# r9y9/gantts

Measured on NVIDIA H100. Metric: gan_step_frames_per_sec, higher is better.
Workload: dtype f32 (GEMMs: bf16x3 split on wgmma, fp32 accumulate)

## Files before the change

### gantts_b200/csrc/gemm_tc.cu

```cuda
#include <cuda.h>
#include <cuda_bf16.h>

#include "common.cuh"
#include "tc_ptx.cuh"

namespace gantts {

constexpr int TC_WG_WARPS = 4;
constexpr int TC_THREADS = 128 + 2 * 32 * TC_WG_WARPS;
constexpr int TC_BM = 128;
constexpr int TC_WARP_PITCH = 20;
constexpr int TC_WARP_BUF_FLOATS = 32 * TC_WARP_PITCH;
constexpr int TC_MAX_BN = 128;
constexpr int TC_KK_BK = 64;
constexpr int TC_MN_BK = 32;
constexpr int TC_MAX_STAGES = 8;
constexpr int TC_PRODUCER_REGS = 40;
constexpr int TC_CONSUMER_REGS = 232;
constexpr uint32_t TC_SMEM_MAX = 227 * 1024;
constexpr uint32_t TC_BIAS_SMEM = 4096;
constexpr uint32_t TC_ONES_SMEM = 1024;

constexpr int EPI_F32 = 0;
constexpr int EPI_PLANES_FWD = 1;
constexpr int EPI_PLANES_BWD = 2;

struct GemmParams {
  int64_t rows_a;
  int cols_b;
  int64_t red;
  int64_t red_chunk;
  int num_a, num_b, num_z;
  int bn;
  int num_stages;
  uint32_t stage_bytes, b_plane_bytes, tx_bytes;
  int64_t row0;
  uint32_t a_plane;
  uint32_t atom_bytes;
  uint32_t epi_off;
  uint32_t bar_off;
  float* C;
  int64_t ldc, c_zstride;
  int vec_ok;
  int accumulate;
  __nv_bfloat16 *out_hi, *out_lo;
  int64_t out_pitch;
  uint32_t* code;
  int64_t code_pitch;
  uint32_t bias_off;
  float* db;
  uint32_t ones_off;
  const float* bias;
  int act;
  float slope, keep_scale;
  uint32_t thresh;
  uint64_t seed;
};

__device__ __forceinline__ uint32_t pack_bf16x2(float a, float b) {
  __nv_bfloat162 h = __floats2bfloat162_rn(a, b);
  return *reinterpret_cast<uint32_t*>(&h);
}

__device__ __forceinline__ void split8(const float* v, uint32_t* h, uint32_t* l) {
#pragma unroll
  for (int i = 0; i < 4; ++i) {
    const float a = v[2 * i], b = v[2 * i + 1];
    const uint32_t hp = pack_bf16x2(a, b);
    const float ah = __uint_as_float(hp << 16), bh = __uint_as_float(hp & 0xffff0000u);
    h[i] = hp;
    l[i] = pack_bf16x2(a - ah, b - bh);
  }
}

__device__ __forceinline__ void store_planes16(const float* v, __nv_bfloat16* hi, __nv_bfloat16* lo, int col,
                                               int64_t pitch) {
  uint32_t h[8], l[8];
  split8(v, h, l);
  split8(v + 8, h + 4, l + 4);
  if (col + 16 <= pitch) {
    reinterpret_cast<uint4*>(hi)[0] = make_uint4(h[0], h[1], h[2], h[3]);
    reinterpret_cast<uint4*>(hi)[1] = make_uint4(h[4], h[5], h[6], h[7]);
    reinterpret_cast<uint4*>(lo)[0] = make_uint4(l[0], l[1], l[2], l[3]);
    reinterpret_cast<uint4*>(lo)[1] = make_uint4(l[4], l[5], l[6], l[7]);
  } else if (col + 8 <= pitch) {
    *reinterpret_cast<uint4*>(hi) = make_uint4(h[0], h[1], h[2], h[3]);
    *reinterpret_cast<uint4*>(lo) = make_uint4(l[0], l[1], l[2], l[3]);
  }
}

__device__ __forceinline__ void dropout16(float (&v)[16], uint64_t seed, uint32_t row, int n_cols, int col, uint32_t thresh,
                                          float scale) {
  const uint32_t quarter_n = (uint32_t)(n_cols + 3) >> 2, limit = drop_limit(thresh);
#pragma unroll
  for (int q = 0; q < 4; ++q) {
    const DropBits d = dropout_quad_bits(seed, row, quarter_n, ((uint32_t)col >> 2) + q);
    v[4 * q] = (d.a << 16) > limit ? v[4 * q] * scale : 0.f;
    v[4 * q + 1] = d.a > limit ? v[4 * q + 1] * scale : 0.f;
    v[4 * q + 2] = (d.b << 16) > limit ? v[4 * q + 2] * scale : 0.f;
    v[4 * q + 3] = d.b > limit ? v[4 * q + 3] * scale : 0.f;
  }
}

__device__ __forceinline__ void epilogue_f32_smem(const GemmParams& p, const uint32_t (&r)[16], int64_t row0,
                                                  int lane, int col, int z, const float* __restrict__ bias_s,
                                                  float* scr) {
  const int64_t row = row0 + (lane & 15);
  const int lcol = col + 16 * (lane >> 4);
  float v[16];
#pragma unroll
  for (int j = 0; j < 16; ++j) v[j] = __uint_as_float(r[j]);
  if (p.bias) {
    if (bias_s) {
#pragma unroll
      for (int j = 0; j < 16; ++j) v[j] += bias_s[lcol + j];
    } else {
#pragma unroll
      for (int j = 0; j < 16; ++j)
        if (lcol + j < p.cols_b) v[j] += __ldg(p.bias + lcol + j);
    }
  }
  if (p.act == GANTTS_ACT_LEAKY_DROPOUT) {
#pragma unroll
    for (int j = 0; j < 16; ++j) v[j] = fmaxf(v[j], v[j] * p.slope);
    if (p.thresh) dropout16(v, p.seed, (uint32_t)(row + p.row0), p.cols_b, lcol, p.thresh, p.keep_scale);
  } else if (p.act == GANTTS_ACT_SIGMOID) {
#pragma unroll
    for (int j = 0; j < 16; ++j) v[j] = 1.f / (1.f + expf(-v[j]));
  }
  const int sw = (lane >> 1) & 3;
#pragma unroll
  for (int k = 0; k < 4; ++k)
    *reinterpret_cast<float4*>(scr + lane * 16 + 4 * (k ^ sw)) = make_float4(v[4 * k], v[4 * k + 1], v[4 * k + 2], v[4 * k + 3]);
  __syncwarp();
  float* cbase = p.C + (int64_t)z * p.c_zstride;
  const int j = lane & 15, hr = lane >> 4;
#pragma unroll
  for (int h = 0; h < 2; ++h) {
    const int c = col + 16 * h + j;
    const bool col_ok = c < p.cols_b;
    float* q[8];
    bool ok[8];
    float old[8];
#pragma unroll
    for (int i = 0; i < 8; ++i) {
      const int64_t rw = row0 + 2 * i + hr;
      q[i] = cbase + c + rw * p.ldc;
      ok[i] = col_ok && rw < p.rows_a;
    }
    if (p.accumulate) {
#pragma unroll
      for (int i = 0; i < 8; ++i) old[i] = ok[i] ? __ldcg(q[i]) : 0.f;
    }
#pragma unroll
    for (int i = 0; i < 8; ++i) {
      const int rr = 2 * (8 * h + i) + hr;
      const float val = scr[rr * 16 + 4 * ((j >> 2) ^ ((rr >> 1) & 3)) + (j & 3)];
      if (ok[i]) *q[i] = p.accumulate ? old[i] + val : val;
    }
  }
  __syncwarp();
}

template <int EPI>
__device__ __forceinline__ uint32_t epilogue_chunk16(const GemmParams& p, const uint32_t (&r)[16], int64_t row,
                                                     int col, int z, const float* __restrict__ bias_s,
                                                     uint32_t code_in) {
  uint32_t code = 0;
  float v[16];
#pragma unroll
  for (int j = 0; j < 16; ++j) v[j] = __uint_as_float(r[j]);
  if (EPI == EPI_F32) {
    float* crow = p.C + (int64_t)z * p.c_zstride + row * p.ldc;
    if (p.bias) {
      if (bias_s) {
#pragma unroll
        for (int j = 0; j < 16; ++j) v[j] += bias_s[col + j];
      } else {
#pragma unroll
        for (int j = 0; j < 16; ++j)
          if (col + j < p.cols_b) v[j] += __ldg(p.bias + col + j);
      }
    }
    if (p.act == GANTTS_ACT_LEAKY_DROPOUT) {
#pragma unroll
      for (int j = 0; j < 16; ++j) v[j] = fmaxf(v[j], v[j] * p.slope);
      if (p.thresh) dropout16(v, p.seed, (uint32_t)(row + p.row0), p.cols_b, col, p.thresh, p.keep_scale);
    } else if (p.act == GANTTS_ACT_SIGMOID) {
#pragma unroll
      for (int j = 0; j < 16; ++j) v[j] = 1.f / (1.f + expf(-v[j]));
    }
#pragma unroll
    for (int j = 0; j < 16; j += 4) {
      const int c = col + j;
      if (c + 3 < p.cols_b) {
        *reinterpret_cast<float4*>(crow + c) = make_float4(v[j], v[j + 1], v[j + 2], v[j + 3]);
      } else {
#pragma unroll
        for (int e = 0; e < 4; ++e)
          if (c + e < p.cols_b) crow[c + e] = v[j + e];
      }
    }
  } else if (EPI == EPI_PLANES_FWD) {
    if (bias_s) {
#pragma unroll
      for (int j = 0; j < 16; j += 4) {
        const float4 b4 = *reinterpret_cast<const float4*>(bias_s + col + j);
        v[j] += b4.x; v[j + 1] += b4.y; v[j + 2] += b4.z; v[j + 3] += b4.w;
      }
    } else {
#pragma unroll
      for (int j = 0; j < 16; ++j)
        if (col + j < p.cols_b) v[j] += __ldg(p.bias + col + j);
    }
    if (p.thresh) {
      const uint32_t quarter_n = (uint32_t)(p.cols_b + 3) >> 2, limit = drop_limit(p.thresh);
      const uint32_t grow = (uint32_t)(row + p.row0);
#pragma unroll
      for (int q = 0; q < 4; ++q) {
        const DropBits d = dropout_quad_bits(p.seed, grow, quarter_n, ((uint32_t)col >> 2) + q);
#pragma unroll
        for (int e = 0; e < 4; ++e) {
          const int j = 4 * q + e;
          const uint32_t w = e < 2 ? d.a : d.b;
          const bool keep = ((e & 1) ? w : (w << 16)) > limit;
          const bool neg = v[j] < 0.f;
          const float a = neg ? v[j] * p.slope : v[j];
          v[j] = keep ? a * p.keep_scale : 0.f;
          if (!keep) code |= 1u << (2 * j);
          if (neg) code |= 2u << (2 * j);
        }
      }
    } else {
#pragma unroll
      for (int j = 0; j < 16; ++j) {
        const bool neg = v[j] < 0.f;
        v[j] = neg ? v[j] * p.slope : v[j];
        if (v[j] == 0.f) code |= 1u << (2 * j);
        if (neg) code |= 2u << (2 * j);
      }
    }
    __nv_bfloat16* oh = p.out_hi + row * p.out_pitch + col;
    __nv_bfloat16* ol = p.out_lo + row * p.out_pitch + col;
    store_planes16(v, oh, ol, col, p.out_pitch);
  } else {
    const float dpos = p.keep_scale, dneg = p.slope * p.keep_scale;
    const float dzero = p.thresh ? 0.f : p.slope;
#pragma unroll
    for (int j = 0; j < 16; ++j) {
      const uint32_t cj = (code_in >> (2 * j)) & 3u;
      v[j] *= (cj & 1u) ? dzero : ((cj & 2u) ? dneg : dpos);
    }
    __nv_bfloat16* oh = p.out_hi + row * p.out_pitch + col;
    __nv_bfloat16* ol = p.out_lo + row * p.out_pitch + col;
    store_planes16(v, oh, ol, col, p.out_pitch);
  }
  return code;
}

template <bool MN, int BN, bool DB>
__device__ __forceinline__ void mma_tile(const GemmParams& p, float (&acc)[BN / 2], float (&accdb)[4], uint32_t base,
                                         uint32_t full0, uint32_t empty0, uint64_t d_ones, int nk, uint32_t& s,
                                         uint32_t& ph, int lane, int blk) {
  constexpr int BK = MN ? TC_MN_BK : TC_KK_BK;
  constexpr uint32_t kstep = MN ? 2048u : 32u;
  const uint32_t a_half = MN ? p.atom_bytes : 8192u;
  const uint32_t a_off = (uint32_t)blk * a_half;
#pragma unroll
  for (int i = 0; i < BN / 2; ++i) acc[i] = 0.f;
  uint32_t prev = 0;
#pragma unroll 1
  for (int kb = 0; kb < nk; ++kb) {
    ptx::mbar_wait(full0 + 8 * s, ph);
    const uint32_t sa_hi = base + s * p.stage_bytes, sa_lo = sa_hi + p.a_plane;
    const uint32_t sb_hi = sa_lo + p.a_plane, sb_lo = sb_hi + p.b_plane_bytes;
    ptx::wgmma_fence();
#pragma unroll
    for (int k = 0; k < BK / 16; ++k) {
      const uint64_t db_hi = ptx::make_smem_desc(sb_hi + k * kstep, p.atom_bytes, 1024u);
      const uint64_t db_lo = ptx::make_smem_desc(sb_lo + k * kstep, p.atom_bytes, 1024u);
      const uint64_t da_hi = ptx::make_smem_desc(sa_hi + a_off + k * kstep, p.atom_bytes, 1024u);
      const uint64_t da_lo = ptx::make_smem_desc(sa_lo + a_off + k * kstep, p.atom_bytes, 1024u);
      if constexpr (BN == 128) {
        ptx::wgmma_m64n128k16<MN ? 1 : 0, MN ? 1 : 0>(acc, da_hi, db_hi);
        ptx::wgmma_m64n128k16<MN ? 1 : 0, MN ? 1 : 0>(acc, da_hi, db_lo);
        ptx::wgmma_m64n128k16<MN ? 1 : 0, MN ? 1 : 0>(acc, da_lo, db_hi);
      } else {
        ptx::wgmma_m64n64k16<MN ? 1 : 0, MN ? 1 : 0>(acc, da_hi, db_hi);
        ptx::wgmma_m64n64k16<MN ? 1 : 0, MN ? 1 : 0>(acc, da_hi, db_lo);
        ptx::wgmma_m64n64k16<MN ? 1 : 0, MN ? 1 : 0>(acc, da_lo, db_hi);
      }
      if constexpr (DB) {
        ptx::wgmma_m64n8k16<MN ? 1 : 0>(accdb, da_hi, d_ones);
        ptx::wgmma_m64n8k16<MN ? 1 : 0>(accdb, da_lo, d_ones);
      }
    }
    ptx::wgmma_commit();
    if (kb > 0) {
      ptx::wgmma_wait<1>();
      __syncwarp();
      if (lane == 0) ptx::mbar_arrive(empty0 + 8 * prev);
    }
    prev = s;
    if (++s == (uint32_t)p.num_stages) { s = 0; ph ^= 1; }
  }
  __syncwarp();
  ptx::wgmma_wait<0>();
  ptx::fence_regs(acc);
  ptx::fence_regs(accdb);
  __syncwarp();
  if (lane == 0) ptx::mbar_arrive(empty0 + 8 * prev);
}

template <bool MN, int EPI, int BN>
__global__ void __launch_bounds__(TC_THREADS, 1)
gemm_bf16x3_kernel(const __grid_constant__ CUtensorMap tmAh, const __grid_constant__ CUtensorMap tmAl,
                   const __grid_constant__ CUtensorMap tmBh, const __grid_constant__ CUtensorMap tmBl,
                   const GemmParams p) {
  constexpr int BK = MN ? TC_MN_BK : TC_KK_BK;
  extern __shared__ uint8_t smem_raw[];
  const uint32_t raw = ptx::smem_u32(smem_raw);
  const uint32_t base = (raw + 1023u) & ~1023u;
  uint8_t* const gbase = smem_raw + (base - raw);
  const uint32_t full0 = base + p.bar_off, empty0 = full0 + 8 * TC_MAX_STAGES;
  const int warp = threadIdx.x >> 5, lane = threadIdx.x & 31;
  const int tiles_ab = p.num_a * p.num_b;
  const int tiles = tiles_ab * p.num_z;
  auto k_blocks = [&](int z) {
    const int64_t r_beg = (int64_t)z * p.red_chunk;
    const int64_t r_end = r_beg + p.red_chunk < p.red ? r_beg + p.red_chunk : p.red;
    return (int)((r_end - r_beg + BK - 1) / BK);
  };

  if (threadIdx.x == 0) {
    for (int s = 0; s < p.num_stages; ++s) {
      ptx::mbar_init(full0 + 8 * s, 1);
      ptx::mbar_init(empty0 + 8 * s, 2 * TC_WG_WARPS);
    }
    ptx::fence_barrier_init();
    ptx::prefetch_tensormap(&tmAh);
    ptx::prefetch_tensormap(&tmAl);
    ptx::prefetch_tensormap(&tmBh);
    ptx::prefetch_tensormap(&tmBl);
  }
  ptx::pdl_launch_dependents();
  ptx::pdl_wait();
  const float* bias_s = nullptr;
  if (p.bias_off) {
    float* bs = reinterpret_cast<float*>(gbase + p.bias_off);
    const int nb = p.num_b * BN;
    for (int i = threadIdx.x; i < nb; i += TC_THREADS) bs[i] = i < p.cols_b ? p.bias[i] : 0.f;
    bias_s = bs;
  }
  if (MN && p.db != nullptr) {
    uint32_t* ones = reinterpret_cast<uint32_t*>(gbase + p.ones_off);
    for (int i = threadIdx.x; i < (int)(TC_ONES_SMEM / 4); i += TC_THREADS) ones[i] = 0x3F803F80u;
    ptx::fence_proxy_async();
  }
  __syncthreads();

  if (warp < 4) {
    ptx::setmaxnreg_dec<TC_PRODUCER_REGS>();
    if (threadIdx.x == 0) {
      uint32_t s = 0, ph = 0;
      for (int t = blockIdx.x; t < tiles; t += gridDim.x) {
        const int z = t / tiles_ab, rem = t - z * tiles_ab;
        const int a0 = (rem / p.num_b) * TC_BM, b0 = (rem % p.num_b) * BN;
        const int64_t r_beg = (int64_t)z * p.red_chunk;
        const int nk = k_blocks(z);
        for (int kb = 0; kb < nk; ++kb) {
          const int64_t r0 = r_beg + (int64_t)kb * BK;
          ptx::mbar_wait(empty0 + 8 * s, ph ^ 1);
          const uint32_t fb = full0 + 8 * s;
          ptx::mbar_expect_tx(fb, p.tx_bytes);
          const uint32_t sa_hi = base + s * p.stage_bytes, sa_lo = sa_hi + p.a_plane;
          const uint32_t sb_hi = sa_lo + p.a_plane, sb_lo = sb_hi + p.b_plane_bytes;
          if (!MN) {
            ptx::tma_load_2d(sa_hi, &tmAh, fb, (int32_t)r0, a0);
            ptx::tma_load_2d(sb_hi, &tmBh, fb, (int32_t)r0, b0);
            ptx::tma_load_2d(sa_lo, &tmAl, fb, (int32_t)r0, a0);
            ptx::tma_load_2d(sb_lo, &tmBl, fb, (int32_t)r0, b0);
          } else {
            for (int j = 0; j < TC_BM / 64; ++j) {
              ptx::tma_load_2d(sa_hi + j * p.atom_bytes, &tmAh, fb, a0 + 64 * j, (int32_t)r0);
              ptx::tma_load_2d(sa_lo + j * p.atom_bytes, &tmAl, fb, a0 + 64 * j, (int32_t)r0);
            }
            for (int j = 0; j < BN / 64; ++j) {
              ptx::tma_load_2d(sb_hi + j * p.atom_bytes, &tmBh, fb, b0 + 64 * j, (int32_t)r0);
              ptx::tma_load_2d(sb_lo + j * p.atom_bytes, &tmBl, fb, b0 + 64 * j, (int32_t)r0);
            }
          }
          if (++s == (uint32_t)p.num_stages) { s = 0; ph ^= 1; }
        }
      }
    }
    return;
  }

  ptx::setmaxnreg_inc<TC_CONSUMER_REGS>();
  const int wg = (warp >> 2) - 1;
  const int q = warp & 3;
  float* const wbuf = reinterpret_cast<float*>(gbase + p.epi_off) + (warp - 4) * TC_WARP_BUF_FLOATS;
  const uint64_t d_ones = ptx::make_smem_desc(base + p.ones_off, 0u, 1024u);
  uint32_t s = 0, ph = 0;
  for (int t = blockIdx.x; t < tiles; t += gridDim.x) {
    const int z = t / tiles_ab, rem = t - z * tiles_ab;
    const int nk = k_blocks(z);
    const int ta = rem / p.num_b, tb = rem % p.num_b;
    const int a0 = ta * TC_BM, b0 = tb * BN;
    float acc[BN / 2];
    float accdb[4] = {0.f, 0.f, 0.f, 0.f};
    const bool do_db = MN && p.db != nullptr && tb == 0;
    if (do_db)
      mma_tile<MN, BN, MN>(p, acc, accdb, base, full0, empty0, d_ones, nk, s, ph, lane, wg);
    else
      mma_tile<MN, BN, false>(p, acc, accdb, base, full0, empty0, d_ones, nk, s, ph, lane, wg);
    const int64_t row0 = (int64_t)a0 + 64 * wg + 16 * q;
    if (do_db && (lane & 3) == 0) {
      const int64_t r = row0 + (lane >> 2);
      if (r < p.rows_a) p.db[(int64_t)z * p.rows_a + r] = accdb[0];
      if (r + 8 < p.rows_a) p.db[(int64_t)z * p.rows_a + r + 8] = accdb[2];
    }
    const int64_t row = row0 + (lane & 15);
    const bool row_ok = row < p.rows_a;
    constexpr int PASSES = BN / 32;
    uint32_t codes[PASSES];
    uint32_t code_out[PASSES];
#pragma unroll
    for (int k = 0; k < PASSES; ++k) {
      const int c = b0 + 16 * (2 * k + (lane >> 4));
      codes[k] = code_out[k] = 0u;
      if (EPI == EPI_PLANES_BWD && row_ok && c < p.cols_b) codes[k] = __ldg(p.code + row * p.code_pitch + (c >> 4));
    }
#pragma unroll
    for (int k = 0; k < PASSES; ++k) {
      __syncwarp();
#pragma unroll
      for (int h = 0; h < 2; ++h)
#pragma unroll
        for (int jj = 0; jj < 2; ++jj) {
          const int j = 2 * (2 * k + h) + jj;
          float* w = wbuf + (16 * h + (lane >> 2)) * TC_WARP_PITCH + 8 * jj + 2 * (lane & 3);
          *reinterpret_cast<float2*>(w) = make_float2(acc[4 * j], acc[4 * j + 1]);
          *reinterpret_cast<float2*>(w + 8 * TC_WARP_PITCH) = make_float2(acc[4 * j + 2], acc[4 * j + 3]);
        }
      __syncwarp();
      uint32_t rr[16];
      const float4* src = reinterpret_cast<const float4*>(wbuf + lane * TC_WARP_PITCH);
#pragma unroll
      for (int m = 0; m < 4; ++m) {
        const float4 f = src[m];
        rr[4 * m] = __float_as_uint(f.x); rr[4 * m + 1] = __float_as_uint(f.y);
        rr[4 * m + 2] = __float_as_uint(f.z); rr[4 * m + 3] = __float_as_uint(f.w);
      }
      const int col = b0 + 32 * k;
      const int lcol = col + 16 * (lane >> 4);
      if (EPI == EPI_F32 && !p.vec_ok) {
        __syncwarp();
        if (col < p.cols_b) epilogue_f32_smem(p, rr, row0, lane, col, z, bias_s, wbuf);
      } else if (row_ok && lcol < p.cols_b) {
        code_out[k] = epilogue_chunk16<EPI>(p, rr, row, lcol, z, bias_s, codes[k]);
      }
    }
    if (EPI == EPI_PLANES_FWD && p.code != nullptr && row_ok) {
      uint32_t* cpp = p.code + row * p.code_pitch + (b0 >> 4);
#pragma unroll
      for (int k = 0; k < PASSES; ++k) {
        const int ck = 2 * k + (lane >> 4);
        if (b0 + 16 * ck < p.cols_b) cpp[ck] = code_out[k];
      }
    }
  }
}

__global__ void split_planes_kernel(const float* __restrict__ src, int64_t rs, int64_t rows, int cols,
                                    __nv_bfloat16* __restrict__ hi, __nv_bfloat16* __restrict__ lo,
                                    int64_t pitch, int transpose) {
  pdl_entry();
  const int lane = threadIdx.x & 31;
  const int64_t warp = ((int64_t)blockIdx.x * blockDim.x + threadIdx.x) >> 5;
  const int64_t nwarps = ((int64_t)gridDim.x * blockDim.x) >> 5;
  if (!transpose) {
    for (int64_t r = warp; r < rows; r += nwarps) {
      const float* sr = src + r * rs;
      uint32_t* hr = reinterpret_cast<uint32_t*>(hi + r * pitch);
      uint32_t* lr = reinterpret_cast<uint32_t*>(lo + r * pitch);
#pragma unroll 2
      for (int c = 2 * lane; c < cols; c += 64) {
        const float a = sr[c], b = (c + 1 < cols) ? sr[c + 1] : 0.f;
        const uint32_t hp = pack_bf16x2(a, b);
        const float ah = __uint_as_float(hp << 16), bh = __uint_as_float(hp & 0xffff0000u);
        hr[c >> 1] = hp;
        lr[c >> 1] = pack_bf16x2(a - ah, b - bh);
      }
    }
  } else {
    for (int64_t r = warp; r < rows; r += nwarps)
      for (int c = lane; c < cols; c += 32) {
        const float v = src[r * rs + c];
        const __nv_bfloat16 h = __float2bfloat16_rn(v);
        hi[(int64_t)c * pitch + r] = h;
        lo[(int64_t)c * pitch + r] = __float2bfloat16_rn(v - __bfloat162float(h));
      }
  }
}

__global__ void splitk_reduce_kernel(const float* __restrict__ partial, int nsplit, int64_t n,
                                     float* __restrict__ out, int accumulate);

typedef CUresult (*EncodeTiledFn)(CUtensorMap*, CUtensorMapDataType, cuuint32_t, void*, const cuuint64_t*,
                                  const cuuint64_t*, const cuuint32_t*, const cuuint32_t*,
                                  CUtensorMapInterleave, CUtensorMapSwizzle, CUtensorMapL2promotion,
                                  CUtensorMapFloatOOBfill);

static EncodeTiledFn get_encode() {
  static EncodeTiledFn fn = nullptr;
  if (!fn) {
    void* p = nullptr;
    cudaDriverEntryPointQueryResult q;
    if (cudaGetDriverEntryPoint("cuTensorMapEncodeTiled", &p, cudaEnableDefault, &q) == cudaSuccess &&
        q == cudaDriverEntryPointSuccess)
      fn = reinterpret_cast<EncodeTiledFn>(p);
  }
  return fn;
}

static int make_map(CUtensorMap* m, const void* ptr, int64_t rows, int64_t cols, int64_t pitch, int box_rows) {
  EncodeTiledFn enc = get_encode();
  if (!enc) {
    set_error("tc: cuTensorMapEncodeTiled entry point unavailable");
    return GANTTS_E_CUDA;
  }
  cuuint64_t dims[2] = {(cuuint64_t)cols, (cuuint64_t)rows};
  cuuint64_t strides[1] = {(cuuint64_t)pitch * 2};
  cuuint32_t box[2] = {64u, (cuuint32_t)box_rows};
  cuuint32_t estr[2] = {1, 1};
  CUresult r = enc(m, CU_TENSOR_MAP_DATA_TYPE_BFLOAT16, 2, const_cast<void*>(ptr), dims, strides, box, estr,
                   CU_TENSOR_MAP_INTERLEAVE_NONE, CU_TENSOR_MAP_SWIZZLE_128B,
                   CU_TENSOR_MAP_L2_PROMOTION_L2_256B,
                   CU_TENSOR_MAP_FLOAT_OOB_FILL_NONE);
  if (r != CUDA_SUCCESS) {
    set_error("tc: cuTensorMapEncodeTiled failed (%d) rows=%lld cols=%lld pitch=%lld box_rows=%d", (int)r,
              (long long)rows, (long long)cols, (long long)pitch, box_rows);
    return GANTTS_E_CUDA;
  }
  return GANTTS_OK;
}

static int current_device() {
  int dev = -1;
  if (cudaGetDevice(&dev) != cudaSuccess) return -1;
  return dev;
}

static int num_sms() {
  static int n[64] = {};
  const int dev = current_device();
  if (dev < 0 || dev >= 64) return 132;
  if (!n[dev]) {
    cudaDeviceGetAttribute(&n[dev], cudaDevAttrMultiProcessorCount, dev);
    if (n[dev] <= 0) n[dev] = 132;
  }
  return n[dev];
}

static inline int64_t pitch_for(int64_t cols) { return (cols + 15) / 16 * 16; }
static inline size_t plane_bytes(int64_t rows, int64_t cols) {
  return ((size_t)rows * pitch_for(cols) * 2 + 255) / 256 * 256;
}

struct Planes {
  __nv_bfloat16 *hi, *lo;
  int64_t rows, cols, pitch;
};

static Planes carve_planes(char*& cur, int64_t rows, int64_t cols) {
  Planes pl;
  pl.rows = rows;
  pl.cols = cols;
  pl.pitch = pitch_for(cols);
  pl.hi = reinterpret_cast<__nv_bfloat16*>(cur);
  cur += plane_bytes(rows, cols);
  pl.lo = reinterpret_cast<__nv_bfloat16*>(cur);
  cur += plane_bytes(rows, cols);
  return pl;
}

static int launch_split(const float* src, int64_t rs, int64_t rows, int cols, const Planes& pl, int transpose,
                        cudaStream_t st) {
  int64_t total = rows * cols;
  int nb = (int)((total + 1023) / 1024);
  if (nb > num_sms() * 8) nb = num_sms() * 8;
  if (nb < 1) nb = 1;
  GANTTS_PDL_LAUNCH((split_planes_kernel), nb, 256, 0, st, src, rs, rows, cols, pl.hi, pl.lo, pl.pitch, transpose);
  GANTTS_LAUNCH_CHECK("split_planes_kernel");
  return GANTTS_OK;
}

static int pick_bn(int n) {
  int bn = (n + 63) / 64 * 64;
  if (bn <= TC_MAX_BN) return bn;
  int tiles = (n + TC_MAX_BN - 1) / TC_MAX_BN;
  bn = ((n + tiles - 1) / tiles + 63) / 64 * 64;
  return bn;
}

struct EpiArgs {
  int epi = EPI_F32;
  float* C = nullptr;
  int64_t ldc = 0;
  int accumulate = 0;
  __nv_bfloat16 *out_hi = nullptr, *out_lo = nullptr;
  int64_t out_pitch = 0;
  uint32_t* code = nullptr;
  int64_t code_pitch = 0;
  const float* bias = nullptr;
  int act = GANTTS_ACT_NONE;
  float slope = 0.f, p = 0.f;
  uint64_t seed = 0;
  int64_t row0 = 0;
};

static void fill_epilogue(GemmParams& p, const EpiArgs& e) {
  p.C = e.C;
  p.ldc = e.ldc;
  p.accumulate = e.accumulate;
  p.vec_ok = (!e.accumulate && e.C && (e.ldc & 3) == 0 && (reinterpret_cast<uintptr_t>(e.C) & 15) == 0) ? 1 : 0;
  p.out_hi = e.out_hi;
  p.out_lo = e.out_lo;
  p.out_pitch = e.out_pitch;
  p.code = e.code;
  p.code_pitch = e.code_pitch;
  p.bias = e.bias;
  p.act = e.act;
  p.slope = e.slope;
  p.keep_scale = e.p > 0.f ? 1.f / (1.f - e.p) : 1.f;
  p.thresh = e.p > 0.f ? (uint32_t)(e.p * 65536.f + 0.5f) : 0u;
  p.seed = e.seed;
  p.row0 = e.row0;
}

static size_t plan_smem(GemmParams& p, const EpiArgs& e) {
  const uint32_t epi = 2 * TC_WG_WARPS * TC_WARP_BUF_FLOATS * 4;
  const uint32_t fixed = 1024 + epi + TC_ONES_SMEM + TC_BIAS_SMEM + 256;
  p.num_stages = (int)((TC_SMEM_MAX - fixed) / p.stage_bytes);
  if (p.num_stages > TC_MAX_STAGES) p.num_stages = TC_MAX_STAGES;
  p.epi_off = (uint32_t)p.num_stages * p.stage_bytes;
  p.ones_off = p.epi_off + epi;
  p.bias_off = (e.bias && (size_t)p.num_b * p.bn * sizeof(float) <= TC_BIAS_SMEM) ? p.ones_off + TC_ONES_SMEM : 0u;
  p.bar_off = p.ones_off + TC_ONES_SMEM + TC_BIAS_SMEM;
  return (size_t)p.bar_off + 256 + 1024;
}

template <bool MN, int EPI, int BN>
static int launch_kernel(const CUtensorMap& mAh, const CUtensorMap& mAl, const CUtensorMap& mBh,
                         const CUtensorMap& mBl, const GemmParams& p, size_t smem, cudaStream_t st) {
  if (smem > TC_SMEM_MAX) {
    set_error("gemm: shared-memory plan of %zu bytes exceeds %u", smem, TC_SMEM_MAX);
    return GANTTS_E_UNSUPPORTED;
  }
  if (p.num_stages < 2) {
    set_error("gemm: shared-memory plan leaves %d ring stage(s), the mainloop needs 2", p.num_stages);
    return GANTTS_E_UNSUPPORTED;
  }
  static bool attr[64] = {};
  const int dev = current_device();
  if (dev < 0 || dev >= 64 || !attr[dev]) {
    GANTTS_CUDA(cudaFuncSetAttribute(gemm_bf16x3_kernel<MN, EPI, BN>, cudaFuncAttributeMaxDynamicSharedMemorySize,
                                     (int)TC_SMEM_MAX));
    if (dev >= 0 && dev < 64) attr[dev] = true;
  }
  const int tiles = p.num_a * p.num_b * p.num_z;
  const int grid = tiles < num_sms() ? tiles : num_sms();
  prof_begin(MN ? PROF_GEMM_MN : PROF_GEMM_KK, 2.0 * (double)p.rows_a * p.cols_b * (double)p.red, st);
  GANTTS_PDL_LAUNCH((gemm_bf16x3_kernel<MN, EPI, BN>), (unsigned)grid, TC_THREADS, smem, st, mAh, mAl, mBh, mBl, p);
  prof_end(st);
  GANTTS_LAUNCH_CHECK("gemm_bf16x3_kernel");
  return GANTTS_OK;
}

template <bool MN, int EPI>
static int launch_bn(const CUtensorMap& mAh, const CUtensorMap& mAl, const CUtensorMap& mBh, const CUtensorMap& mBl,
                     const GemmParams& p, size_t smem, cudaStream_t st) {
  if (p.bn == 64) return launch_kernel<MN, EPI, 64>(mAh, mAl, mBh, mBl, p, smem, st);
  return launch_kernel<MN, EPI, 128>(mAh, mAl, mBh, mBl, p, smem, st);
}

static int launch_gemm_kk(const Planes& A, const Planes& B, const EpiArgs& e, cudaStream_t st) {
  GemmParams p{};
  p.rows_a = A.rows;
  p.cols_b = (int)B.rows;
  p.red = A.cols;
  if (B.cols != A.cols) {
    set_error("gemm_kk: reduction extents differ (%lld vs %lld)", (long long)A.cols, (long long)B.cols);
    return GANTTS_E_BADARG;
  }
  p.a_plane = TC_BM * 128u;
  p.red_chunk = (p.red + TC_KK_BK - 1) / TC_KK_BK * TC_KK_BK;
  p.bn = pick_bn(p.cols_b);
  p.num_a = (int)((p.rows_a + TC_BM - 1) / TC_BM);
  p.num_b = (p.cols_b + p.bn - 1) / p.bn;
  p.num_z = 1;
  p.b_plane_bytes = (uint32_t)p.bn * 128u;
  p.stage_bytes = 2 * p.a_plane + 2 * p.b_plane_bytes;
  p.tx_bytes = p.stage_bytes;
  p.c_zstride = 0;
  fill_epilogue(p, e);
  const size_t smem = plan_smem(p, e);
  CUtensorMap mAh, mAl, mBh, mBl;
  int rc;
  if ((rc = make_map(&mAh, A.hi, A.rows, A.cols, A.pitch, TC_BM))) return rc;
  if ((rc = make_map(&mAl, A.lo, A.rows, A.cols, A.pitch, TC_BM))) return rc;
  if ((rc = make_map(&mBh, B.hi, B.rows, B.cols, B.pitch, p.bn))) return rc;
  if ((rc = make_map(&mBl, B.lo, B.rows, B.cols, B.pitch, p.bn))) return rc;
  switch (e.epi) {
    case EPI_F32: return launch_bn<false, EPI_F32>(mAh, mAl, mBh, mBl, p, smem, st);
    case EPI_PLANES_FWD: return launch_bn<false, EPI_PLANES_FWD>(mAh, mAl, mBh, mBl, p, smem, st);
    case EPI_PLANES_BWD: return launch_bn<false, EPI_PLANES_BWD>(mAh, mAl, mBh, mBl, p, smem, st);
  }
  set_error("gemm_kk: bad epilogue %d", e.epi);
  return GANTTS_E_BADARG;
}

static size_t mn_partial_bytes(int64_t red, int rows_a, int cols_b, int* splits_out, int64_t* chunk_out) {
  int bn = pick_bn(cols_b);
  int tiles = ((rows_a + TC_BM - 1) / TC_BM) * ((cols_b + bn - 1) / bn);
  const int bk = TC_MN_BK;
  int64_t blocks = (red + bk - 1) / bk;
  int64_t splits = num_sms() / tiles;
  if (splits < 1) splits = 1;
  if (splits > blocks) splits = blocks;
  int64_t chunk = (blocks + splits - 1) / splits * bk;
  splits = (red + chunk - 1) / chunk;
  if (splits_out) *splits_out = (int)splits;
  if (chunk_out) *chunk_out = chunk;
  return ((size_t)splits * ((size_t)rows_a * cols_b + rows_a) * sizeof(float) + 255) / 256 * 256;
}

static size_t mn_partial_bytes_upto(int64_t red_max, int rows_a, int cols_b) {
  const int bn = pick_bn(cols_b);
  const int tiles = ((rows_a + TC_BM - 1) / TC_BM) * ((cols_b + bn - 1) / bn);
  const int64_t blocks = (red_max + TC_MN_BK - 1) / TC_MN_BK;
  int64_t splits = num_sms() / tiles;
  if (splits > blocks) splits = blocks;
  if (splits < 1) splits = 1;
  return ((size_t)splits * ((size_t)rows_a * cols_b + rows_a) * sizeof(float) + 255) / 256 * 256;
}

constexpr int REDUCE_MAX_JOBS = 2 * GANTTS_MAX_LAYERS;
struct ReduceList {
  int n = 0;
  const float* partial[REDUCE_MAX_JOBS];
  float* out[REDUCE_MAX_JOBS];
  int splits[REDUCE_MAX_JOBS];
  int64_t len[REDUCE_MAX_JOBS];
  int64_t off[REDUCE_MAX_JOBS + 1];
};

constexpr int MR_WARPS = 8;
__global__ void __launch_bounds__(32 * MR_WARPS) multi_reduce_kernel(ReduceList rl, int accumulate) {
  pdl_entry();
  __shared__ float4 part_s[MR_WARPS][32];
  const int lane = threadIdx.x & 31, w = threadIdx.x >> 5;
  const int64_t total4 = rl.off[rl.n];
  for (int64_t base = (int64_t)blockIdx.x * 32; base < total4; base += (int64_t)gridDim.x * 32) {
    const int64_t i = base + lane;
    int j = 0;
    float4 s = make_float4(0.f, 0.f, 0.f, 0.f);
    int64_t e = 0, n = 0;
    bool vec = false;
    if (i < total4) {
// ... 45 lines not shown

static int flush_reduce(ReduceList& rl, int accumulate, cudaStream_t st) {
  if (rl.n == 0) return GANTTS_OK;
  rl.off[0] = 0;
  for (int j = 0; j < rl.n; ++j) rl.off[j + 1] = rl.off[j] + (rl.len[j] + 3) / 4;
  int64_t nb = (rl.off[rl.n] + 31) / 32;
  if (nb > (int64_t)num_sms() * 16) nb = (int64_t)num_sms() * 16;
  GANTTS_PDL_LAUNCH((multi_reduce_kernel), (unsigned)nb, 32 * MR_WARPS, 0, st, rl, accumulate);
  GANTTS_LAUNCH_CHECK("multi_reduce_kernel");
  rl.n = 0;
  return GANTTS_OK;
}

static int launch_gemm_mn(const Planes& A, const Planes& B, float* C, float* gb, int accumulate, float* partial,
                          cudaStream_t st, ReduceList* defer = nullptr) {
  GemmParams p{};
  p.rows_a = A.cols;
  p.cols_b = (int)B.cols;
  p.red = A.rows;
  if (B.rows != A.rows) {
    set_error("gemm_mn: reduction extents differ (%lld vs %lld)", (long long)A.rows, (long long)B.rows);
    return GANTTS_E_BADARG;
  }
  int splits;
  int64_t chunk;
  mn_partial_bytes(p.red, (int)p.rows_a, p.cols_b, &splits, &chunk);
  p.red_chunk = chunk;
  p.num_z = splits;
  p.bn = pick_bn(p.cols_b);
  p.num_a = (int)((p.rows_a + TC_BM - 1) / TC_BM);
  p.num_b = (p.cols_b + p.bn - 1) / p.bn;
  p.atom_bytes = (uint32_t)TC_MN_BK * 128;
  p.a_plane = (TC_BM / 64) * p.atom_bytes;
  p.b_plane_bytes = (uint32_t)(p.bn / 64) * p.atom_bytes;
  p.stage_bytes = 2 * p.a_plane + 2 * p.b_plane_bytes;
  p.tx_bytes = p.stage_bytes;
  const bool direct = (splits == 1 && !accumulate);
  const int64_t n = (int64_t)p.rows_a * p.cols_b;
  float* db_partial = partial + (int64_t)splits * n;
  EpiArgs e;
  e.epi = EPI_F32;
  e.C = direct ? C : partial;
  e.ldc = p.cols_b;
  fill_epilogue(p, e);
  p.c_zstride = n;
  p.db = gb ? (direct ? gb : db_partial) : nullptr;
  const size_t smem = plan_smem(p, e);
  CUtensorMap mAh, mAl, mBh, mBl;
  int rc;
  if ((rc = make_map(&mAh, A.hi, A.rows, A.cols, A.pitch, TC_MN_BK))) return rc;
  if ((rc = make_map(&mAl, A.lo, A.rows, A.cols, A.pitch, TC_MN_BK))) return rc;
  if ((rc = make_map(&mBh, B.hi, B.rows, B.cols, B.pitch, TC_MN_BK))) return rc;
  if ((rc = make_map(&mBl, B.lo, B.rows, B.cols, B.pitch, TC_MN_BK))) return rc;
  if ((rc = launch_bn<true, EPI_F32>(mAh, mAl, mBh, mBl, p, smem, st))) return rc;
  if (!direct) {
    if (defer && defer->n + 2 <= REDUCE_MAX_JOBS) {
      int j = defer->n++;
      defer->partial[j] = partial; defer->out[j] = C; defer->splits[j] = splits; defer->len[j] = n;
      if (gb) {
        j = defer->n++;
        defer->partial[j] = db_partial; defer->out[j] = gb; defer->splits[j] = splits; defer->len[j] = p.rows_a;
      }
      return GANTTS_OK;
    }
    splitk_reduce_kernel<<<(unsigned)((n + 1023) / 1024), 256, 0, st>>>(partial, splits, n, C, accumulate);
    GANTTS_LAUNCH_CHECK("splitk_reduce_kernel(tc gW)");
    if (gb) {
      splitk_reduce_kernel<<<(unsigned)((p.rows_a + 1023) / 1024), 256, 0, st>>>(db_partial, splits, p.rows_a, gb,
                                                                               accumulate);
      GANTTS_LAUNCH_CHECK("splitk_reduce_kernel(tc gb)");
    }
  }
  return GANTTS_OK;
}

size_t tc_linear_workspace_bytes(int64_t M, int N, int K) {
  size_t fwd = 2 * plane_bytes(M, K) + 2 * plane_bytes(N, K);
  size_t bwd = 2 * plane_bytes(M, N) + 2 * plane_bytes(M, K) + 2 * plane_bytes(K, N) +
               mn_partial_bytes(M, N, K, nullptr, nullptr) + 256;
  return (fwd > bwd ? fwd : bwd) + 1024;
}

int tc_linear_fwd(const float* x, int64_t x_rs, const float* W, const float* bias, float* y, int64_t y_rs,
                  int64_t M, int N, int K, int act, float slope, float p, uint64_t seed, void* ws,
                  size_t ws_bytes, cudaStream_t st) {
  size_t need = tc_linear_workspace_bytes(M, N, K);
  if (!ws || ws_bytes < need) {
    set_error("tc_linear_fwd: workspace too small (%zu < %zu)", ws_bytes, need);
    return GANTTS_E_WORKSPACE;
  }
  char* cur = reinterpret_cast<char*>((reinterpret_cast<uintptr_t>(ws) + 255) / 256 * 256);
  Planes X = carve_planes(cur, M, K), Wp = carve_planes(cur, N, K);
  int rc;
  if ((rc = launch_split(x, x_rs, M, K, X, 0, st))) return rc;
  if ((rc = launch_split(W, K, N, K, Wp, 0, st))) return rc;
  EpiArgs e;
  e.epi = EPI_F32;
  e.C = y;
  e.ldc = y_rs;
  e.bias = bias;
  e.act = act;
  e.slope = slope;
  e.p = act == GANTTS_ACT_LEAKY_DROPOUT ? p : 0.f;
  e.seed = seed;
  return launch_gemm_kk(X, Wp, e, st);
}

// ... 32 lines not shown
```

### gantts_b200/csrc/tc_ptx.cuh

```cuda
#pragma once
#include <cuda.h>
#include <cuda_runtime.h>
#include <stdint.h>
#include <stdio.h>

namespace gantts {
namespace ptx {

__device__ __forceinline__ uint32_t smem_u32(const void* p) {
  return static_cast<uint32_t>(__cvta_generic_to_shared(p));
}

__device__ __forceinline__ void mbar_init(uint32_t bar, uint32_t count) {
  asm volatile("mbarrier.init.shared::cta.b64 [%0], %1;" ::"r"(bar), "r"(count) : "memory");
}
__device__ __forceinline__ void fence_barrier_init() {
  asm volatile("fence.mbarrier_init.release.cluster;" ::: "memory");
}
__device__ __forceinline__ void fence_proxy_async() {
  asm volatile("fence.proxy.async.shared::cta;" ::: "memory");
}
__device__ __forceinline__ void mbar_expect_tx(uint32_t bar, uint32_t bytes) {
  asm volatile("mbarrier.arrive.expect_tx.shared::cta.b64 _, [%0], %1;" ::"r"(bar), "r"(bytes) : "memory");
}
__device__ __forceinline__ void mbar_arrive(uint32_t bar) {
  asm volatile("mbarrier.arrive.shared::cta.b64 _, [%0];" ::"r"(bar) : "memory");
}
__device__ __forceinline__ bool mbar_try_wait(uint32_t bar, uint32_t parity) {
  uint32_t ok;
  asm volatile(
      "{\n\t.reg .pred P1;\n\t"
      "mbarrier.try_wait.parity.shared::cta.b64 P1, [%1], %2;\n\t"
      "selp.u32 %0, 1, 0, P1;\n\t}\n"
      : "=r"(ok)
      : "r"(bar), "r"(parity)
      : "memory");
  return ok != 0;
}
__device__ __forceinline__ void mbar_wait(uint32_t bar, uint32_t parity) {
  if (mbar_try_wait(bar, parity)) return;
  const long long t0 = clock64();
  while (!mbar_try_wait(bar, parity)) {
    if (clock64() - t0 > 4000000000LL) __trap();
  }
}

__device__ __forceinline__ void prefetch_tensormap(const CUtensorMap* m) {
  asm volatile("prefetch.tensormap [%0];" ::"l"(reinterpret_cast<uint64_t>(m)) : "memory");
}
__device__ __forceinline__ void tma_load_2d(uint32_t dst, const CUtensorMap* map, uint32_t bar, int32_t c0,
                                            int32_t c1) {
  asm volatile(
      "cp.async.bulk.tensor.2d.shared::cluster.global.mbarrier::complete_tx::bytes [%0], [%1, {%3, %4}], [%2];"
      ::"r"(dst), "l"(reinterpret_cast<uint64_t>(map)), "r"(bar), "r"(c0), "r"(c1)
      : "memory");
}

__device__ __forceinline__ void pdl_launch_dependents() { asm volatile("griddepcontrol.launch_dependents;" ::: "memory"); }
__device__ __forceinline__ void pdl_wait() { asm volatile("griddepcontrol.wait;" ::: "memory"); }

template <int R>
__device__ __forceinline__ void setmaxnreg_dec() { asm volatile("setmaxnreg.dec.sync.aligned.u32 %0;" ::"n"(R)); }
template <int R>
__device__ __forceinline__ void setmaxnreg_inc() { asm volatile("setmaxnreg.inc.sync.aligned.u32 %0;" ::"n"(R)); }

__device__ __forceinline__ uint64_t make_smem_desc(uint32_t smem_addr, uint32_t lbo_bytes, uint32_t sbo_bytes) {
  uint64_t d = 0;
  d |= static_cast<uint64_t>((smem_addr >> 4) & 0x3fffu);
  d |= static_cast<uint64_t>((lbo_bytes >> 4) & 0x3fffu) << 16;
  d |= static_cast<uint64_t>((sbo_bytes >> 4) & 0x3fffu) << 32;
  d |= static_cast<uint64_t>(1) << 62;
  return d;
}

__device__ __forceinline__ void wgmma_fence() { asm volatile("wgmma.fence.sync.aligned;" ::: "memory"); }
__device__ __forceinline__ void wgmma_commit() { asm volatile("wgmma.commit_group.sync.aligned;" ::: "memory"); }
template <int N>
__device__ __forceinline__ void wgmma_wait() { asm volatile("wgmma.wait_group.sync.aligned %0;" ::"n"(N) : "memory"); }
template <int R>
__device__ __forceinline__ void fence_regs(float (&d)[R]) {
#pragma unroll
  for (int i = 0; i < R; ++i) asm volatile("" : "+f"(d[i])::"memory");
}

template <int TA, int TB>
__device__ __forceinline__ void wgmma_m64n64k16(float (&d)[32], uint64_t da, uint64_t db) {
  asm volatile(
      "{\n\t.reg .pred p;\n\t"
      "setp.ne.b32 p, 1, 0;\n\t"
      "wgmma.mma_async.sync.aligned.m64n64k16.f32.bf16.bf16 "
      "{%0, %1, %2, %3, %4, %5, %6, %7, %8, %9, %10, %11, %12, %13, %14, %15, "
      "%16, %17, %18, %19, %20, %21, %22, %23, %24, %25, %26, %27, %28, %29, %30, %31}, "
      "%32, %33, p, 1, 1, %34, %35;\n\t}\n"
      : "+f"(d[0]), "+f"(d[1]), "+f"(d[2]), "+f"(d[3]), "+f"(d[4]), "+f"(d[5]), "+f"(d[6]), "+f"(d[7]),
        "+f"(d[8]), "+f"(d[9]), "+f"(d[10]), "+f"(d[11]), "+f"(d[12]), "+f"(d[13]), "+f"(d[14]), "+f"(d[15]),
        "+f"(d[16]), "+f"(d[17]), "+f"(d[18]), "+f"(d[19]), "+f"(d[20]), "+f"(d[21]), "+f"(d[22]), "+f"(d[23]),
        "+f"(d[24]), "+f"(d[25]), "+f"(d[26]), "+f"(d[27]), "+f"(d[28]), "+f"(d[29]), "+f"(d[30]), "+f"(d[31])
      : "l"(da), "l"(db), "n"(TA), "n"(TB));
}
template <int TA, int TB>
__device__ __forceinline__ void wgmma_m64n128k16(float (&d)[64], uint64_t da, uint64_t db) {
  asm volatile(
      "{\n\t.reg .pred p;\n\t"
      "setp.ne.b32 p, 1, 0;\n\t"
      "wgmma.mma_async.sync.aligned.m64n128k16.f32.bf16.bf16 "
      "{%0, %1, %2, %3, %4, %5, %6, %7, %8, %9, %10, %11, %12, %13, %14, %15, "
      "%16, %17, %18, %19, %20, %21, %22, %23, %24, %25, %26, %27, %28, %29, %30, %31, "
      "%32, %33, %34, %35, %36, %37, %38, %39, %40, %41, %42, %43, %44, %45, %46, %47, "
      "%48, %49, %50, %51, %52, %53, %54, %55, %56, %57, %58, %59, %60, %61, %62, %63}, "
// ... 24 lines not shown
```

Baseline: 14.80 million.

## Write bf16 hi/lo output planes via per-warp TMA stores instead of direct stores

The planes epilogues now stage each warp's 16x32 hi and lo bf16 tiles in the warp's shared-memory buffer and issue 2D TMA bulk-tensor stores, replacing per-thread 16-byte global stores. Stores are software-pipelined: each pass's tile is written while the next pass is computed, with bulk wait_group.read guarding buffer reuse. The backward-pass code loads are also hoisted ahead of the MMA loop so their latency overlaps compute. This adds tensor-map setup and extra shared-memory round trips per pass, and relies on TMA clipping for out-of-range rows and columns.

Result: faster. 15.93 million (median of 6 runs) (+7.6%).

```diff
diff --git a/gantts_b200/csrc/gemm_tc.cu b/gantts_b200/csrc/gemm_tc.cu
--- a/gantts_b200/csrc/gemm_tc.cu
+++ b/gantts_b200/csrc/gemm_tc.cu
@@ -43,7 +43,6 @@
   int64_t ldc, c_zstride;
   int vec_ok;
   int accumulate;
-  __nv_bfloat16 *out_hi, *out_lo;
   int64_t out_pitch;
   uint32_t* code;
   int64_t code_pitch;
@@ -73,19 +72,24 @@
   }
 }
 
-__device__ __forceinline__ void store_planes16(const float* v, __nv_bfloat16* hi, __nv_bfloat16* lo, int col,
-                                               int64_t pitch) {
-  uint32_t h[8], l[8];
-  split8(v, h, l);
-  split8(v + 8, h + 4, l + 4);
-  if (col + 16 <= pitch) {
-    reinterpret_cast<uint4*>(hi)[0] = make_uint4(h[0], h[1], h[2], h[3]);
-    reinterpret_cast<uint4*>(hi)[1] = make_uint4(h[4], h[5], h[6], h[7]);
-    reinterpret_cast<uint4*>(lo)[0] = make_uint4(l[0], l[1], l[2], l[3]);
-    reinterpret_cast<uint4*>(lo)[1] = make_uint4(l[4], l[5], l[6], l[7]);
-  } else if (col + 8 <= pitch) {
-    *reinterpret_cast<uint4*>(hi) = make_uint4(h[0], h[1], h[2], h[3]);
-    *reinterpret_cast<uint4*>(lo) = make_uint4(l[0], l[1], l[2], l[3]);
+__device__ __forceinline__ void store_planes_pass(const CUtensorMap* mh, const CUtensorMap* ml, float* buf,
+                                                  const uint32_t (&h)[8], const uint32_t (&l)[8], int lane, int col,
+                                                  int64_t row0, const GemmParams& p) {
+  if (lane == 0) ptx::bulk_wait_read<0>();
+  __syncwarp();
+  uint4* sh = reinterpret_cast<uint4*>(reinterpret_cast<uint8_t*>(buf) + (lane & 15) * 64 + (lane >> 4) * 32);
+  uint4* sl = sh + 1024 / 16;
+  sh[0] = make_uint4(h[0], h[1], h[2], h[3]);
+  sh[1] = make_uint4(h[4], h[5], h[6], h[7]);
+  sl[0] = make_uint4(l[0], l[1], l[2], l[3]);
+  sl[1] = make_uint4(l[4], l[5], l[6], l[7]);
+  ptx::fence_proxy_async();
+  __syncwarp();
+  if (lane == 0 && row0 < p.rows_a && col < p.out_pitch) {
+    const uint32_t s = ptx::smem_u32(buf);
+    ptx::tma_store_2d(mh, s, col, (int32_t)row0);
+    ptx::tma_store_2d(ml, s + 1024, col, (int32_t)row0);
+    ptx::bulk_commit();
   }
 }
 
@@ -165,7 +169,7 @@
 template <int EPI>
 __device__ __forceinline__ uint32_t epilogue_chunk16(const GemmParams& p, const uint32_t (&r)[16], int64_t row,
                                                      int col, int z, const float* __restrict__ bias_s,
-                                                     uint32_t code_in) {
+                                                     uint32_t code_in, uint32_t (&h)[8], uint32_t (&l)[8]) {
   uint32_t code = 0;
   float v[16];
 #pragma unroll
@@ -240,9 +244,8 @@
         if (neg) code |= 2u << (2 * j);
       }
     }
-    __nv_bfloat16* oh = p.out_hi + row * p.out_pitch + col;
-    __nv_bfloat16* ol = p.out_lo + row * p.out_pitch + col;
-    store_planes16(v, oh, ol, col, p.out_pitch);
+    split8(v, h, l);
+    split8(v + 8, h + 4, l + 4);
   } else {
     const float dpos = p.keep_scale, dneg = p.slope * p.keep_scale;
     const float dzero = p.thresh ? 0.f : p.slope;
@@ -251,9 +254,8 @@
       const uint32_t cj = (code_in >> (2 * j)) & 3u;
       v[j] *= (cj & 1u) ? dzero : ((cj & 2u) ? dneg : dpos);
     }
-    __nv_bfloat16* oh = p.out_hi + row * p.out_pitch + col;
-    __nv_bfloat16* ol = p.out_lo + row * p.out_pitch + col;
-    store_planes16(v, oh, ol, col, p.out_pitch);
+    split8(v, h, l);
+    split8(v + 8, h + 4, l + 4);
   }
   return code;
 }
@@ -316,8 +318,10 @@
 __global__ void __launch_bounds__(TC_THREADS, 1)
 gemm_bf16x3_kernel(const __grid_constant__ CUtensorMap tmAh, const __grid_constant__ CUtensorMap tmAl,
                    const __grid_constant__ CUtensorMap tmBh, const __grid_constant__ CUtensorMap tmBl,
+                   const __grid_constant__ CUtensorMap tmOh, const __grid_constant__ CUtensorMap tmOl,
                    const GemmParams p) {
   constexpr int BK = MN ? TC_MN_BK : TC_KK_BK;
+  constexpr bool PLANES = EPI != EPI_F32;
   extern __shared__ uint8_t smem_raw[];
   const uint32_t raw = ptx::smem_u32(smem_raw);
   const uint32_t base = (raw + 1023u) & ~1023u;
@@ -342,6 +346,10 @@
     ptx::prefetch_tensormap(&tmAl);
     ptx::prefetch_tensormap(&tmBh);
     ptx::prefetch_tensormap(&tmBl);
+    if (PLANES) {
+      ptx::prefetch_tensormap(&tmOh);
+      ptx::prefetch_tensormap(&tmOl);
+    }
   }
   ptx::pdl_launch_dependents();
   ptx::pdl_wait();
@@ -408,6 +416,17 @@
     const int nk = k_blocks(z);
     const int ta = rem / p.num_b, tb = rem % p.num_b;
     const int a0 = ta * TC_BM, b0 = tb * BN;
+    const int64_t row0 = (int64_t)a0 + 64 * wg + 16 * q;
+    const int64_t row = row0 + (lane & 15);
+    const bool row_ok = row < p.rows_a;
+    constexpr int PASSES = BN / 32;
+    uint32_t codes[PASSES];
+#pragma unroll
+    for (int k = 0; k < PASSES; ++k) {
+      const int c = b0 + 16 * (2 * k + (lane >> 4));
+      codes[k] = 0u;
+      if (EPI == EPI_PLANES_BWD && row_ok && c < p.cols_b) codes[k] = __ldg(p.code + row * p.code_pitch + (c >> 4));
+    }
     float acc[BN / 2];
     float accdb[4] = {0.f, 0.f, 0.f, 0.f};
     const bool do_db = MN && p.db != nullptr && tb == 0;
@@ -415,25 +434,17 @@
       mma_tile<MN, BN, MN>(p, acc, accdb, base, full0, empty0, d_ones, nk, s, ph, lane, wg);
     else
       mma_tile<MN, BN, false>(p, acc, accdb, base, full0, empty0, d_ones, nk, s, ph, lane, wg);
-    const int64_t row0 = (int64_t)a0 + 64 * wg + 16 * q;
     if (do_db && (lane & 3) == 0) {
       const int64_t r = row0 + (lane >> 2);
       if (r < p.rows_a) p.db[(int64_t)z * p.rows_a + r] = accdb[0];
       if (r + 8 < p.rows_a) p.db[(int64_t)z * p.rows_a + r + 8] = accdb[2];
     }
-    const int64_t row = row0 + (lane & 15);
-    const bool row_ok = row < p.rows_a;
-    constexpr int PASSES = BN / 32;
-    uint32_t codes[PASSES];
     uint32_t code_out[PASSES];
+    uint32_t hw[8], lw[8];
 #pragma unroll
     for (int k = 0; k < PASSES; ++k) {
-      const int c = b0 + 16 * (2 * k + (lane >> 4));
-      codes[k] = code_out[k] = 0u;
-      if (EPI == EPI_PLANES_BWD && row_ok && c < p.cols_b) codes[k] = __ldg(p.code + row * p.code_pitch + (c >> 4));
-    }
-#pragma unroll
-    for (int k = 0; k < PASSES; ++k) {
+      code_out[k] = 0u;
+      if (PLANES && lane == 0) ptx::bulk_wait_read<0>();
       __syncwarp();
 #pragma unroll
       for (int h = 0; h < 2; ++h)
@@ -458,10 +469,14 @@
       if (EPI == EPI_F32 && !p.vec_ok) {
         __syncwarp();
         if (col < p.cols_b) epilogue_f32_smem(p, rr, row0, lane, col, z, bias_s, wbuf);
-      } else if (row_ok && lcol < p.cols_b) {
-        code_out[k] = epilogue_chunk16<EPI>(p, rr, row, lcol, z, bias_s, codes[k]);
-      }
-    }
+      } else if (EPI == EPI_F32) {
+        if (row_ok && lcol < p.cols_b) epilogue_chunk16<EPI>(p, rr, row, lcol, z, bias_s, 0u, hw, lw);
+      } else {
+        if (k > 0) store_planes_pass(&tmOh, &tmOl, wbuf, hw, lw, lane, col - 32, row0, p);
+        code_out[k] = epilogue_chunk16<EPI>(p, rr, row, lcol, z, bias_s, codes[k], hw, lw);
+      }
+    }
+    if (PLANES) store_planes_pass(&tmOh, &tmOl, wbuf, hw, lw, lane, b0 + 32 * (PASSES - 1), row0, p);
     if (EPI == EPI_PLANES_FWD && p.code != nullptr && row_ok) {
       uint32_t* cpp = p.code + row * p.code_pitch + (b0 >> 4);
 #pragma unroll
@@ -471,6 +486,7 @@
       }
     }
   }
+  if (PLANES && lane == 0) ptx::bulk_wait<0>();
 }
 
 __global__ void split_planes_kernel(const float* __restrict__ src, int64_t rs, int64_t rows, int cols,
@@ -525,7 +541,8 @@
   return fn;
 }
 
-static int make_map(CUtensorMap* m, const void* ptr, int64_t rows, int64_t cols, int64_t pitch, int box_rows) {
+static int make_map(CUtensorMap* m, const void* ptr, int64_t rows, int64_t cols, int64_t pitch, int box_rows,
+                    int box_cols = 64, CUtensorMapSwizzle swizzle = CU_TENSOR_MAP_SWIZZLE_128B) {
   EncodeTiledFn enc = get_encode();
   if (!enc) {
     set_error("tc: cuTensorMapEncodeTiled entry point unavailable");
@@ -533,10 +550,10 @@
   }
   cuuint64_t dims[2] = {(cuuint64_t)cols, (cuuint64_t)rows};
   cuuint64_t strides[1] = {(cuuint64_t)pitch * 2};
-  cuuint32_t box[2] = {64u, (cuuint32_t)box_rows};
+  cuuint32_t box[2] = {(cuuint32_t)box_cols, (cuuint32_t)box_rows};
   cuuint32_t estr[2] = {1, 1};
   CUresult r = enc(m, CU_TENSOR_MAP_DATA_TYPE_BFLOAT16, 2, const_cast<void*>(ptr), dims, strides, box, estr,
-                   CU_TENSOR_MAP_INTERLEAVE_NONE, CU_TENSOR_MAP_SWIZZLE_128B,
+                   CU_TENSOR_MAP_INTERLEAVE_NONE, swizzle,
                    CU_TENSOR_MAP_L2_PROMOTION_L2_256B,
                    CU_TENSOR_MAP_FLOAT_OOB_FILL_NONE);
   if (r != CUDA_SUCCESS) {
@@ -626,8 +643,6 @@
   p.ldc = e.ldc;
   p.accumulate = e.accumulate;
   p.vec_ok = (!e.accumulate && e.C && (e.ldc & 3) == 0 && (reinterpret_cast<uintptr_t>(e.C) & 15) == 0) ? 1 : 0;
-  p.out_hi = e.out_hi;
-  p.out_lo = e.out_lo;
   p.out_pitch = e.out_pitch;
   p.code = e.code;
   p.code_pitch = e.code_pitch;
@@ -654,7 +669,8 @@
 
 template <bool MN, int EPI, int BN>
 static int launch_kernel(const CUtensorMap& mAh, const CUtensorMap& mAl, const CUtensorMap& mBh,
-                         const CUtensorMap& mBl, const GemmParams& p, size_t smem, cudaStream_t st) {
+                         const CUtensorMap& mBl, const CUtensorMap& mOh, const CUtensorMap& mOl, const GemmParams& p,
+                         size_t smem, cudaStream_t st) {
   if (smem > TC_SMEM_MAX) {
     set_error("gemm: shared-memory plan of %zu bytes exceeds %u", smem, TC_SMEM_MAX);
     return GANTTS_E_UNSUPPORTED;
@@ -673,7 +689,8 @@
   const int tiles = p.num_a * p.num_b * p.num_z;
   const int grid = tiles < num_sms() ? tiles : num_sms();
   prof_begin(MN ? PROF_GEMM_MN : PROF_GEMM_KK, 2.0 * (double)p.rows_a * p.cols_b * (double)p.red, st);
-  GANTTS_PDL_LAUNCH((gemm_bf16x3_kernel<MN, EPI, BN>), (unsigned)grid, TC_THREADS, smem, st, mAh, mAl, mBh, mBl, p);
+  GANTTS_PDL_LAUNCH((gemm_bf16x3_kernel<MN, EPI, BN>), (unsigned)grid, TC_THREADS, smem, st, mAh, mAl, mBh, mBl, mOh,
+                    mOl, p);
   prof_end(st);
   GANTTS_LAUNCH_CHECK("gemm_bf16x3_kernel");
   return GANTTS_OK;
@@ -681,9 +698,10 @@
 
 template <bool MN, int EPI>
 static int launch_bn(const CUtensorMap& mAh, const CUtensorMap& mAl, const CUtensorMap& mBh, const CUtensorMap& mBl,
-                     const GemmParams& p, size_t smem, cudaStream_t st) {
-  if (p.bn == 64) return launch_kernel<MN, EPI, 64>(mAh, mAl, mBh, mBl, p, smem, st);
-  return launch_kernel<MN, EPI, 128>(mAh, mAl, mBh, mBl, p, smem, st);
+                     const CUtensorMap& mOh, const CUtensorMap& mOl, const GemmParams& p, size_t smem,
+                     cudaStream_t st) {
+  if (p.bn == 64) return launch_kernel<MN, EPI, 64>(mAh, mAl, mBh, mBl, mOh, mOl, p, smem, st);
+  return launch_kernel<MN, EPI, 128>(mAh, mAl, mBh, mBl, mOh, mOl, p, smem, st);
 }
 
 static int launch_gemm_kk(const Planes& A, const Planes& B, const EpiArgs& e, cudaStream_t st) {
@@ -713,10 +731,13 @@
   if ((rc = make_map(&mAl, A.lo, A.rows, A.cols, A.pitch, TC_BM))) return rc;
   if ((rc = make_map(&mBh, B.hi, B.rows, B.cols, B.pitch, p.bn))) return rc;
   if ((rc = make_map(&mBl, B.lo, B.rows, B.cols, B.pitch, p.bn))) return rc;
+  if (e.epi == EPI_F32) return launch_bn<false, EPI_F32>(mAh, mAl, mBh, mBl, mAh, mAl, p, smem, st);
+  CUtensorMap mOh, mOl;
+  if ((rc = make_map(&mOh, e.out_hi, p.rows_a, e.out_pitch, e.out_pitch, 16, 32, CU_TENSOR_MAP_SWIZZLE_NONE))) return rc;
+  if ((rc = make_map(&mOl, e.out_lo, p.rows_a, e.out_pitch, e.out_pitch, 16, 32, CU_TENSOR_MAP_SWIZZLE_NONE))) return rc;
   switch (e.epi) {
-    case EPI_F32: return launch_bn<false, EPI_F32>(mAh, mAl, mBh, mBl, p, smem, st);
-    case EPI_PLANES_FWD: return launch_bn<false, EPI_PLANES_FWD>(mAh, mAl, mBh, mBl, p, smem, st);
-    case EPI_PLANES_BWD: return launch_bn<false, EPI_PLANES_BWD>(mAh, mAl, mBh, mBl, p, smem, st);
+    case EPI_PLANES_FWD: return launch_bn<false, EPI_PLANES_FWD>(mAh, mAl, mBh, mBl, mOh, mOl, p, smem, st);
+    case EPI_PLANES_BWD: return launch_bn<false, EPI_PLANES_BWD>(mAh, mAl, mBh, mBl, mOh, mOl, p, smem, st);
   }
   set_error("gemm_kk: bad epilogue %d", e.epi);
   return GANTTS_E_BADARG;
@@ -868,7 +889,7 @@
   if ((rc = make_map(&mAl, A.lo, A.rows, A.cols, A.pitch, TC_MN_BK))) return rc;
   if ((rc = make_map(&mBh, B.hi, B.rows, B.cols, B.pitch, TC_MN_BK))) return rc;
   if ((rc = make_map(&mBl, B.lo, B.rows, B.cols, B.pitch, TC_MN_BK))) return rc;
-  if ((rc = launch_bn<true, EPI_F32>(mAh, mAl, mBh, mBl, p, smem, st))) return rc;
+  if ((rc = launch_bn<true, EPI_F32>(mAh, mAl, mBh, mBl, mAh, mAl, p, smem, st))) return rc;
   if (!direct) {
     if (defer && defer->n + 2 <= REDUCE_MAX_JOBS) {
       int j = defer->n++;
diff --git a/gantts_b200/csrc/tc_ptx.cuh b/gantts_b200/csrc/tc_ptx.cuh
--- a/gantts_b200/csrc/tc_ptx.cuh
+++ b/gantts_b200/csrc/tc_ptx.cuh
@@ -55,6 +55,16 @@
       ::"r"(dst), "l"(reinterpret_cast<uint64_t>(map)), "r"(bar), "r"(c0), "r"(c1)
       : "memory");
 }
+__device__ __forceinline__ void tma_store_2d(const CUtensorMap* map, uint32_t src, int32_t c0, int32_t c1) {
+  asm volatile("cp.async.bulk.tensor.2d.global.shared::cta.bulk_group [%0, {%2, %3}], [%1];"
+               ::"l"(reinterpret_cast<uint64_t>(map)), "r"(src), "r"(c0), "r"(c1)
+               : "memory");
+}
+__device__ __forceinline__ void bulk_commit() { asm volatile("cp.async.bulk.commit_group;" ::: "memory"); }
+template <int N>
+__device__ __forceinline__ void bulk_wait_read() { asm volatile("cp.async.bulk.wait_group.read %0;" ::"n"(N) : "memory"); }
+template <int N>
+__device__ __forceinline__ void bulk_wait() { asm volatile("cp.async.bulk.wait_group %0;" ::"n"(N) : "memory"); }
 
 __device__ __forceinline__ void pdl_launch_dependents() { asm volatile("griddepcontrol.launch_dependents;" ::: "memory"); }
 __device__ __forceinline__ void pdl_wait() { asm volatile("griddepcontrol.wait;" ::: "memory"); }
```
